# raider99k/UNINA-YOLO-DLA

Measured on AMD Instinct MI355X. Metric: frames/sec, 640x640 batch-1 (p99 latency alongside), higher is better.
Workload: dtype f16; 1 GPU; unina-yolo-dla-m graph A fp16, batch=1, 640x640, NMS on-GPU (BASELINE configs[1]); frames_in_flight_per_gpu=2, parallelism=1 GPU, distinct_frames=2048, detections_last_frame=446

## Files before the change

### include/unina_mi355.h

```cpp
#ifndef UNINA_MI355_H
#define UNINA_MI355_H

#include <stddef.h>
#include <stdint.h>

#ifdef UNINA_NO_HIP_HEADERS
typedef struct ihipStream_t *hipStream_t;
typedef int hipError_t;
#else
#include <hip/hip_runtime_api.h>
#endif

#ifdef __cplusplus
extern "C" {
#endif

#define MAX_DETECTIONS 1024

#if defined(__cplusplus)
struct alignas(32) GpuDetection {
#else
struct GpuDetection {
#endif
  float x1, y1, x2, y2;
// ... 275 lines not shown


typedef struct unina_op_info {
  char name[96];
  char kernel[64];
  int kind;
  int m, n, k;
  double flops;
  double bytes;
  int grid, block;
} unina_op_info;

int unina_op_count(const unina_engine_t *e);
int unina_get_op_info(const unina_engine_t *e, int index, unina_op_info *info);

int unina_profile_ops(unina_engine_t *e, int iters, float *ms_per_op, hipStream_t stream);

int unina_profile_post(unina_engine_t *e, int iters, float conf_threshold, float iou_threshold, float conformal_q, float *ms2,
                       hipStream_t stream);

int unina_conv_config_count(void);
const char *unina_conv_config_name(int cfg);
int unina_set_op_config(unina_engine_t *e, int op_index, int cfg);
int unina_autotune(unina_engine_t *e, int iters, hipStream_t stream);

int unina_set_fusion(unina_engine_t *e, int enable);
int unina_fusion_groups(const unina_engine_t *e);
int unina_debug_fusable_groups(const char *path);

int unina_debug_read_buffer(unina_engine_t *e, const char *name, float *host_out, size_t capacity_floats,
                            int *c, int *h, int *w);

int unina_debug_post_stamps(unina_engine_t *e, long long *out16);

int unina_debug_conv_stamps(unina_engine_t *e, int op_index, long long *out5, hipStream_t stream);

int unina_debug_dual_stamps(unina_engine_t *e, int op_index, long long *out16, hipStream_t stream);
int unina_debug_dual_timeline(unina_engine_t* e, int op_index, long long* out, int cap, hipStream_t stream);
int unina_debug_block_stamps(unina_engine_t *e, int op_index, long long *out16, hipStream_t stream);
int unina_debug_folded_heads(unina_engine_t *e);
int unina_debug_owned_streams(void);
int unina_debug_streams_overlap(int device, hipStream_t a, hipStream_t b, int reps, long long *stamps, int *overlapped);

const char *unina_version(void);

#define UNINA_COMM_ID_BYTES 128
typedef struct unina_comm unina_comm;
int unina_comm_unique_id(void *id128);
int unina_comm_init(unina_comm **out, const void *id128, int rank, int world, int device_id);
int unina_comm_all_gather(unina_comm *c, const void *d_send, void *d_recv, size_t bytes_per_rank, hipStream_t stream);
int unina_comm_rank(const unina_comm *c);
int unina_comm_world(const unina_comm *c);
void unina_comm_destroy(unina_comm *c);
const char *unina_comm_last_error(void);

hipError_t init_postprocess_resources(void);
hipError_t cleanup_postprocess_resources(void);
hipError_t reset_detection_counter(hipStream_t stream);
hipError_t get_detection_count(int *count, hipStream_t stream);
hipError_t decode_yolo_head(const float *d_cls, const float *d_reg, GpuDetection *d_detections, int grid_w,
                            int grid_h, int stride, int num_classes, float conf_threshold, float conformal_q,
                            hipStream_t stream);
hipError_t run_gpu_nms(GpuDetection *d_detections, int num_detections, float iou_threshold, hipStream_t stream);
hipError_t copy_valid_detections_to_host(const GpuDetection *d_detections, GpuDetection *h_detections,
                                         int num_detections, int *out_valid_count, hipStream_t stream);

// ... 33 lines not shown
```

### unina-yolo-dla_amd/csrc/engine.hip

```cpp
#include <cstdarg>
#include <cstdio>
#include <atomic>
#include <chrono>
#include <climits>
#include <cstdlib>
#include <cstring>
#include <string>
#include <vector>

#include "calib.h"
#include "engine_format.h"
#include "engine_validate.h"
#include "kernels.h"
#include "mining.h"

using namespace unina;

static_assert(kMaxClasses == (uint32_t)kMaxNumClasses, "the validator's class-count limit is the post-process's class field");

hipError_t unina::kernels_init() {
  for (hipError_t (*init)() : {conv_init, c3k2_init, head_init, pair_init, block_dual_init, stem_pool_init, post_init, calib_init}) {
    const hipError_t e = init();
    if (e != hipSuccess) return e;
  }
// ... 1993 lines not shown
                                 int y_pitch, int uv_pitch, const unina_tile* tiles, int n_tiles, const NormParams* norm,
                                 float conf, float iou, float q, float merge_iou, GpuDetection* d_out, int* d_out_count,
                                 hipStream_t stream) {
  const unina_frame f = nv12_frame(d_y, d_uv, src_width, src_height, y_pitch, uv_pitch);
  return infer_tiled(e, "unina_infer_tiled_nv12", &f, tiles, n_tiles, norm, conf, iou, q, merge_iou, true, d_out, d_out_count, stream);
}

int unina_infer_tiled_nv12(unina_engine_t* e, const uint8_t* d_y, const uint8_t* d_uv, int src_width, int src_height, int y_pitch,
                           int uv_pitch, const unina_tile* tiles, int n_tiles, const NormParams* norm, float conf, float iou,
                           float q, float merge_iou, GpuDetection* out, int* out_count, hipStream_t stream) {
  const unina_frame f = nv12_frame(d_y, d_uv, src_width, src_height, y_pitch, uv_pitch);
  return infer_tiled(e, "unina_infer_tiled_nv12", &f, tiles, n_tiles, norm, conf, iou, q, merge_iou, false, out, out_count, stream);
}

int unina_infer_tiled_frame_async(unina_engine_t* e, const unina_frame* frame, const unina_tile* tiles, int n_tiles, const NormParams* norm,
                                  float conf, float iou, float q, float merge_iou, GpuDetection* d_out, int* d_out_count,
                                  hipStream_t stream) {
  return infer_tiled(e, "unina_infer_tiled_frame_async", frame, tiles, n_tiles, norm, conf, iou, q, merge_iou, true, d_out, d_out_count, stream);
}

int unina_infer_tiled_frame(unina_engine_t* e, const unina_frame* frame, const unina_tile* tiles, int n_tiles, const NormParams* norm,
                            float conf, float iou, float q, float merge_iou, GpuDetection* out, int* out_count, hipStream_t stream) {
  return infer_tiled(e, "unina_infer_tiled_frame", frame, tiles, n_tiles, norm, conf, iou, q, merge_iou, false, out, out_count, stream);
}

int unina_debug_post_stamps(unina_engine_t* e, long long* out16) {
  if (!e || !out16) return UNINA_ERR_ARG;
  HIPCHK(e, hipSetDevice(e->device));
  HIPCHK(e, hipDeviceSynchronize());
  HIPCHK(e, hipMemcpy(out16, e->d_result->pad_stamps, sizeof(long long) * 16, hipMemcpyDeviceToHost));
  return UNINA_OK;
}

int unina_debug_conv_stamps(unina_engine_t* e, int op_index, long long* out5, hipStream_t stream) {
  if (!e || !out5 || op_index < 0 || op_index >= (int)e->ops.size()) return UNINA_ERR_ARG;
  HIPCHK(e, hipSetDevice(e->device));
  if (e->plan_dirty) {
    int rc = plan(e);
    if (rc != UNINA_OK) return rc;
  }
  if (e->ops[op_index].d.kind != kOpConv) return fail(e, UNINA_ERR_ARG, "op %d is not a convolution", op_index);
  long long* stamps = reinterpret_cast<long long*>(e->d_result->pad_stamps);
  HIPCHK(e, hipMemsetAsync(stamps, 0, sizeof(long long) * 8, stream));
  HIPCHK(e, launch_op_as(e, op_index, stream, kLaunchConv, [&](OpLaunch& l) { l.cp[0].stamps = stamps; }));
  HIPCHK(e, hipStreamSynchronize(stream));
  HIPCHK(e, hipMemcpy(out5, stamps, sizeof(long long) * 8, hipMemcpyDeviceToHost));
  return UNINA_OK;
}

int unina_debug_dual_stamps(unina_engine_t* e, int op_index, long long* out16, hipStream_t stream) {
  if (!e || !out16 || op_index < 0 || op_index >= (int)e->ops.size()) return UNINA_ERR_ARG;
  HIPCHK(e, hipSetDevice(e->device));
  if (e->plan_dirty) {
    int rc = plan(e);
    if (rc != UNINA_OK) return rc;
  }
  const PlannedOp& op = e->ops[op_index];
  if (op.d.kind != kOpConv || op.fuse_role || op.dual_with < 0 || op.dual_absorbed)
    return fail(e, UNINA_ERR_ARG, "op %d does not lead a dual conv launch", op_index);
  long long* stamps = reinterpret_cast<long long*>(e->d_result->pad_stamps);
  HIPCHK(e, hipMemsetAsync(stamps, 0, sizeof(long long) * 16, stream));
  HIPCHK(e, launch_op_as(e, op_index, stream, kLaunchConvDual, [&](OpLaunch& l) {
    l.cp[0].stamps = stamps;
    l.cp[1].stamps = stamps + 8;
  }));
  HIPCHK(e, hipStreamSynchronize(stream));
// ... 269 lines not shown
```

### unina-yolo-dla_amd/csrc/kernels.h

```cpp
#pragma once
#include <hip/hip_runtime.h>
#include <cstdint>
#include <vector>

#include "../../include/unina_mi355.h"
#include "camera_source.h"

namespace unina {

typedef _Float16 half_t;
enum DType : int { kF16 = 0, kF32 = 1, kI8 = 2, kS16 = 3 };
constexpr int kNumDTypes = 4;
struct s16_t { _Float16 v; };

struct LaunchDesc {
  const void* func;
  dim3 grid, block;
  unsigned shmem;
  const char* name;
};
inline hipError_t launch_desc(const LaunchDesc& d, void** args, hipStream_t stream) {
  return hipLaunchKernel(d.func, d.grid, d.block, args, d.shmem, stream);
}

// ... 195 lines not shown
  void* buf;
  long long lo;
  int H, W, C, ld, coff;
};
hipError_t sppf_pool_desc(const PoolParams& p, LaunchDesc* d);

struct QuantParams {
  const half_t* src;
  signed char* dst;
  size_t n;
  float inv_scale;
};
hipError_t quant_desc(const QuantParams& p, LaunchDesc* d);

struct CandList {
  GpuDetection* cand;
  uint2* ke;
  int* hist;
  int* total;
};
enum PostMode { kPostOneLaunch = 0, kPostSplit = 1 };
enum PostStamp {
  kStampDecoded = 0,
  kStampHandoff = 1, kStampListRead = 1,
  kStampGathered = 2,
  kStampSorted = 3, kStampNmsStart = 3,
  kStampMasks = 4, kStampTilesDone = 4,
  kStampScanned = 5,
  kStampOutput = 6,
  kStampDecodeStart = 7,
  kStampLoaded = 8,
  kStampLists = 9,
  kStampScanWave0 = 10,
  kPostStampCount = 14
};
struct PostParams {
  const float* cls[3];
  const float* reg[3];
  int gw[3], gh[3], stride[3];
  int num_classes;
  float conf_thr, iou_thr, conformal_q;
  GpuDetection* cand;
  int* block_count;
  unsigned int* ticket;
  GpuDetection* out;
  int* out_count;
  int* out_candidates;
  long long* stamps;
  unsigned int* done_flag;
  unsigned int done_value;
  PostMode mode;
  CandList list;
  float4* ws_box;
  float2* ws_cc;
  unsigned int* ticket2;
  int eoff[3];
  int* ws_rank;
  unsigned long long* ws_full;
  unsigned long long* ws_rownz;
  const void* h1[3];
  long long h1_lo[3];
  int h1_ld[3], h1_c[3];
  int h1_coff[3][2];
  const unsigned char* w2[3][2];
  const float* b2[3][2];
  int bstart[4];
  int cpb[3];
// ... 27 lines not shown
```

### unina-yolo-dla_amd/csrc/postprocess.hip

```cpp
#include "kernels.h"
#include "mfma_common.h"
#include "post_math.h"
#include "wave_block.h"

#pragma clang fp contract(off)

namespace unina {

namespace {

constexpr int kT = kPostBlock;
constexpr int kWaves = kT / 64;
constexpr int kMaxDet = MAX_DETECTIONS;
constexpr int kWords = kMaxDet / 64;
constexpr int kTriWords = 64 * (kWords * (kWords + 1) / 2);

struct Smem {
  int scan[kT + 8];
  unsigned long long keys[kMaxDet];
  float4 box[kMaxDet];
  float2 cc[kMaxDet];
  unsigned long long mask[kTriWords];
  unsigned long long rownz[kWords];
  unsigned long long removed[kWords];
// ... 438 lines not shown

namespace {

constexpr int kT2 = kPost2Block;
constexpr int kW2 = kT2 / 64;

struct SmemD {
  float stage[32][kT2];
  int wave_cnt[kW2];
  int run0;
};

constexpr int kTN = 512;
constexpr int kWN = kTN / 64;
constexpr int kColsPerWave = 64 / kWN;
constexpr int kMemCap = 1024;
struct SelectScratch {
  int hist[kBins];
  unsigned mkey[kMemCap];
  int meidx[kMemCap];
  int mpos[kMemCap];
  int part[kTN];
};
struct SmemN {
  float4 rbox[64], cbox[64];
  float2 rcc[64], ccc[64];
  unsigned char piece[64][kWN];
  unsigned char rcnt[64][kWN];
  union {
    unsigned long long mask[kMaxDet * kWords];
    SelectScratch sel;
  };
  unsigned short perm[kMaxDet];
  unsigned short list[4][kMaxDet];
  unsigned long long removed[4][kWords];
  unsigned long long rownz[kWords];
  int misc[4];
  int wave_cnt[kWN];
  int sel_cnt[kWN];
  int is_last;
};
static_assert(sizeof(SelectScratch) <= sizeof(unsigned long long) * kMaxDet * kWords, "select_top's scratch lives in the mask's LDS");
static_assert(kClassMask == kMaxNumClasses, "the all-ones class field is the dummy's -1");

__device__ __forceinline__ int list_reserve(const CandList& l, int count) {
  return count ? __hip_atomic_fetch_add(l.total, count, __ATOMIC_RELAXED, __HIP_MEMORY_SCOPE_AGENT) : 0;
}
__device__ __forceinline__ void list_put(const CandList& l, int at, uint4 box, uint4 rest, unsigned eidx) {
  uint4* dst = reinterpret_cast<uint4*>(l.cand + at);
  dst[0] = box;
  dst[1] = make_uint4(rest.x, rest.y, rest.z, eidx);
  l.ke[at] = make_uint2(rest.x, eidx);
  const int bin = conf_bin(__uint_as_float(rest.x));
  atomicAdd(&l.hist[bin < 0 ? 0 : bin], 1);
}

}

__global__ __launch_bounds__(kPost2Block) void post_decode_kernel(const PostParams p) {
  SmemD& s = *reinterpret_cast<SmemD*>(post_smem);
  const int tid = threadIdx.x, lane = tid & 63, wv = tid >> 6;
  const int b = blockIdx.x;
  const int h = b < p.bstart[1] ? 0 : (b < p.bstart[2] ? 1 : 2);
  const int cpb = p.cpb[h];
  const int cell0 = (b - p.bstart[h]) * cpb;
  const int gw = p.gw[h], ncell = gw * p.gh[h];
  const int idx = cell0 + tid;
  stamp(p.stamps, kStampDecodeStart, true);
  bool pass = false;
// ... 261 lines not shown
    st_sc1(p.ws_cc + c * 64 + tid, s.rcc[tid]);
  }
  const int gi = c * 64 + lane;
  const float4 a = s.rbox[lane];
  const float2 ac = s.rcc[lane];
  const float area_a = (a.z - a.x) * (a.w - a.y);
  unsigned int rowbits = 0u;
  int rowcnt = 0, colcnt = 0;
  unsigned long long colword = 0ull;
#pragma unroll
  for (int u = 0; u < kColsPerWave; ++u) {
    const int col = wv * kColsPerWave + u;
    const int gj = w * 64 + col;
    const float4 bb = s.cbox[col];
    const float2 bc = s.ccc[col];
    const bool j_first = bc.x > ac.x || (bc.x == ac.x && ce_eidx(bc.y) < ce_eidx(ac.y));
    const bool i_first = gi != gj && !j_first;
    const bool over = gi != gj && ce_same_class(bc.y, ac.y) && iou_exceeds(a, area_a, bb, p.iou_thr);
    if (over && ac.x > bc.x) rowbits |= 1u << u;
    rowcnt += j_first ? 1 : 0;
    const unsigned long long cw = __ballot(over && bc.x > ac.x);
    const int cc = __popcll(__ballot(i_first));
    if (lane == u) {
      colword = cw;
      colcnt = cc;
    }
  }
  s.piece[lane][wv] = (unsigned char)rowbits;
  s.rcnt[lane][wv] = (unsigned char)rowcnt;
  const unsigned long long colnz = __ballot(lane < kColsPerWave && colword != 0ull);
  if (w != c) {
    if (lane < kColsPerWave) {
      const int gj = w * 64 + wv * kColsPerWave + lane;
      st_sc1(p.ws_full + (size_t)gj * kWords + c, colword);
      atomicAdd(&p.ws_rank[gj], colcnt);
    }
    if (lane == 0 && colnz) atomicOr(&p.ws_rownz[w], colnz << (kColsPerWave * wv));
  }
  __syncthreads();
  if (tid < 64) {
    unsigned long long word = 0ull;
    int cnt = 0;
#pragma unroll
    for (int v = 0; v < kWN; ++v) {
      word |= (unsigned long long)s.piece[tid][v] << (kColsPerWave * v);
      cnt += s.rcnt[tid][v];
    }
    st_sc1(p.ws_full + (size_t)gi * kWords + w, word);
    atomicAdd(&p.ws_rank[gi], cnt);
    const unsigned long long nz = __ballot(word != 0ull);
    if (tid == 0 && nz) atomicOr(&p.ws_rownz[c], nz);
  }
}

struct OwnCands {
  int rk[2];
  float2 cc[2];
  float4 bx[2];
};

__device__ __forceinline__ OwnCands load_ranks_and_masks(SmemN& s, const PostParams& p, int n, int nw) {
  const int tid = threadIdx.x;
  constexpr int B = 8;
  const int words = n * nw;
  OwnCands o;
#pragma unroll
  for (int q = 0; q < 2; ++q) {
    const int e = tid + q * kTN;
    o.rk[q] = e < n ? __hip_atomic_load(p.ws_rank + e, __ATOMIC_RELAXED, __HIP_MEMORY_SCOPE_AGENT) : 0;
    o.cc[q] = e < n ? ld_sc1(p.ws_cc + e) : make_float2(0.f, 0.f);
    o.bx[q] = e < n ? ld_sc1(p.ws_box + e) : make_float4(0.f, 0.f, 0.f, 0.f);
  }
  unsigned long long rz = tid < kWords ? __hip_atomic_load(p.ws_rownz + tid, __ATOMIC_RELAXED, __HIP_MEMORY_SCOPE_AGENT) : 0ull;
  for (int k0 = tid; k0 < words; k0 += kTN * B) {
    unsigned long long v[B];
#pragma unroll
    for (int q = 0; q < B; ++q) {
      const int k = k0 + q * kTN;
      const int row = k / nw, wd = k - row * nw;
      v[q] = k < words ? ld_sc1(p.ws_full + (size_t)row * kWords + wd) : 0ull;
    }
#pragma unroll
    for (int q = 0; q < B; ++q) {
      const int k = k0 + q * kTN;
      if (k < words) s.mask[k] = v[q];
    }
  }
  if (tid < kWords) s.rownz[tid] = rz;
  __syncthreads();
#pragma unroll
  for (int q = 0; q < 2; ++q) {
    const int e = tid + q * kTN;
    if (e < n && (unsigned)o.rk[q] < (unsigned)n) {
      const unsigned nz = (unsigned)((s.rownz[e >> 6] >> (e & 63)) & 1ull);
      s.perm[o.rk[q]] = (unsigned short)(e | ((__float_as_int(o.cc[q].y) & 3) << 10) | (nz << 12));
    }
  }
  __syncthreads();
  return o;
}

__device__ __forceinline__ void class_split_scan(SmemN& s, long long* stamps, int n, int nw) {
  const int tid = threadIdx.x, lane = tid & 63, wv = tid >> 6;
  if (wv < 4) {
    unsigned long long removed_reg = 0ull;
    int m = 0;
    for (int r0 = 0; r0 < n; r0 += 64) {
      const int r = r0 + lane;
      const int ent = r < n ? (int)s.perm[r] : 0;
      const bool take = r < n && (ent >> 12) && ((ent >> 10) & 3) == wv;
      const unsigned long long bal = __ballot(take);
      if (take) s.list[wv][m + __popcll(bal & ((1ull << lane) - 1ull))] = (unsigned short)(ent & 1023);
      m += __popcll(bal);
    }
    asm volatile("s_waitcnt lgkmcnt(0)" ::: "memory");
    stamp(stamps, kStampLists);
    if (stamps && lane == 0) stamps[kStampScanWave0 + wv] = m;
    for (int k0 = 0; k0 < m; k0 += 64) {
      const int cnt = m - k0 < 64 ? m - k0 : 64;
      const int mine = k0 + lane < m ? (int)s.list[wv][k0 + lane] : 0;
      for (int kb = 0; kb < cnt; kb += 16) {
        unsigned long long pre[16];
#pragma unroll
        for (int q = 0; q < 16; ++q) {
          const int iq = __builtin_amdgcn_readlane(mine, (kb + q) & 63);
          pre[q] = lane < nw ? s.mask[iq * nw + lane] : 0ull;
        }
#pragma unroll
        for (int q = 0; q < 16; ++q) {
          const int i = __builtin_amdgcn_readlane(mine, (kb + q) & 63);
          const unsigned long long cur = lane_word(removed_reg, i >> 6);
          const bool act = kb + q < cnt && !((cur >> (i & 63)) & 1ull);
          removed_reg |= act ? pre[q] : 0ull;
        }
      }
    }
    if (lane < kWords) s.removed[wv][lane] = removed_reg;
    if (stamps && lane == 0) stamps[kStampScanWave0 + wv] |= (long long)(wall_clock64() & 0xFFFFFFFFll) << 20;
  }
  __syncthreads();
  if (tid < kWords) s.removed[0][tid] |= s.removed[1][tid] | s.removed[2][tid] | s.removed[3][tid];
  __syncthreads();
}

__device__ __forceinline__ void emit_and_reset(SmemN& s, const PostParams& p, int n, int nw, int total, const OwnCands& o) {
  const int tid = threadIdx.x;
  int base = 0;
#pragma unroll
  for (int q = 0; q < 2; ++q) {
    const int r = tid + q * kTN;
    if (q * kTN >= n) break;
    bool kept = false;
    if (r < n) {
      const int i = s.perm[r] & 1023;
      kept = !((s.removed[0][i >> 6] >> (i & 63)) & 1ull);
    }
    int tot;
    const int at = base + block_rank<kWN>(kept, s.wave_cnt, &tot);
    if (r < n) s.list[0][r] = (unsigned short)at;
    base += tot;
  }
  __syncthreads();
#pragma unroll
  for (int q = 0; q < 2; ++q) {
    const int e = tid + q * kTN;
    if (e < n && (unsigned)o.rk[q] < (unsigned)n && !((s.removed[0][e >> 6] >> (e & 63)) & 1ull)) {
      GpuDetection d = make_det(o.bx[q], o.cc[q].x, ce_class(o.cc[q].y), 1);
      map_box(p, d);
      p.out[s.list[0][o.rk[q]]] = d;
    }
  }
  for (int e = tid; e < nw * 64; e += kTN) p.ws_rank[e] = 0;
  if (tid < kWords) p.ws_rownz[tid] = 0ull;
  for (int i = tid; i < kBins; i += kTN) p.list.hist[i] = 0;
  if (tid == 0) {
    *p.out_count = base;
    if (p.out_candidates) *p.out_candidates = total;
    __hip_atomic_store(p.list.total, 0, __ATOMIC_RELAXED, __HIP_MEMORY_SCOPE_AGENT);
    __hip_atomic_store(p.ticket2, 0u, __ATOMIC_RELAXED, __HIP_MEMORY_SCOPE_AGENT);
  }
}

}

__global__ __launch_bounds__(kTN) void post_nms_kernel(const PostParams p) {
  SmemN& s = *reinterpret_cast<SmemN*>(post_smem);
  stamp(p.stamps, kStampNmsStart, true);
  const int total = __hip_atomic_load(p.list.total, __ATOMIC_RELAXED, __HIP_MEMORY_SCOPE_AGENT);
  stamp(p.stamps, kStampListRead, true);
  const int n = total < kMaxDet ? total : kMaxDet;
  const int nw = (n + 63) >> 6;
  const int ntiles = nw * (nw + 1) / 2;
  const int t = blockIdx.x;
  if (t >= (ntiles > 0 ? ntiles : 1)) return;
  if (ntiles > 0) {
    const TileCW tile = tile_of(t, nw);
    fetch_tile(s, p, total, n, tile);
    stamp(p.stamps, kStampGathered, true);
    pair_tile(s, p, tile);
    if (!arrive_and_check_last_sc1(p.ticket2, &s.is_last, ntiles)) return;
  }
  stamp(p.stamps, kStampTilesDone);
  const OwnCands own = load_ranks_and_masks(s, p, n, nw);
  stamp(p.stamps, kStampLoaded);
  class_split_scan(s, p.stamps, n, nw);
  stamp(p.stamps, kStampScanned);
  emit_and_reset(s, p, n, nw, total, own);
  stamp(p.stamps, kStampOutput);
  signal_done(p, threadIdx.x);
}

__global__ __launch_bounds__(kPost2Block) void tile_gather_kernel(const TileGatherParams g) {
  int& s_base = *reinterpret_cast<int*>(post_smem);
  const int t = blockIdx.x, tid = threadIdx.x;
  int cnt = g.counts[t];
  cnt = cnt < 0 ? 0 : (cnt > kMaxDet ? kMaxDet : cnt);
  if (tid == 0) s_base = list_reserve(g.list, cnt);
  __syncthreads();
  const int base = s_base;
  const TileMap m = g.map[t];
  const uint4* src = reinterpret_cast<const uint4*>(g.slots + (size_t)t * kMaxDet);
  for (int i = tid; i < cnt; i += kPost2Block) {
    const uint4 bx = src[2 * i], rest = src[2 * i + 1];
    const float x1 = __uint_as_float(bx.x) * m.sx + m.ox, y1 = __uint_as_float(bx.y) * m.sy + m.oy;
    const float x2 = __uint_as_float(bx.z) * m.sx + m.ox, y2 = __uint_as_float(bx.w) * m.sy + m.oy;
    list_put(g.list, base + i, make_uint4(__float_as_uint(x1), __float_as_uint(y1), __float_as_uint(x2), __float_as_uint(y2)), rest,
             (unsigned)(t * kMaxDet + i));
  }
}

int post_num_blocks(const int gw[3], const int gh[3]) {
  const int cells = gw[0] * gh[0] + gw[1] * gh[1] + gw[2] * gh[2];
  return (cells + kPostBlock - 1) / kPostBlock;
}

constexpr size_t kListCap = 256 * 1024;
static_assert(kListCap == (size_t)1 << (32 - kClassBits), "an enumeration index must fit the bits above the class in pack_ce");
size_t post_workspace_bytes() {
  return sizeof(float4) * kMaxDet + sizeof(float2) * kMaxDet + 256 + sizeof(int) * kBins + sizeof(uint2) * kListCap +
         sizeof(int) * kMaxDet + sizeof(unsigned long long) * ((size_t)kMaxDet * kWords + kWords);
// ... 237 lines not shown
```

### unina-yolo-dla_amd/engine.py

```python
from __future__ import annotations

import ctypes as C
import os
import tempfile
from typing import Dict, List, Optional

import numpy as np

from . import export as _export
from .graph import Graph, OUTPUT_NAMES

_PKG = os.path.dirname(os.path.abspath(__file__))
LIB_PATH = os.environ.get("UNINA_LIB") or os.path.join(_PKG, "libunina_mi355.so")
MAX_DETECTIONS = 1024

DET_DTYPE = np.dtype([("x1", "<f4"), ("y1", "<f4"), ("x2", "<f4"), ("y2", "<f4"), ("confidence", "<f4"),
                      ("class_id", "<i4"), ("valid", "<i4"), ("_pad", "<i4")])
assert DET_DTYPE.itemsize == 32

ERRORS = {1: "IO", 2: "FORMAT", 3: "HIP", 4: "ARG", 5: "STATE", 6: "UNSUPPORTED"}


class OpInfo(C.Structure):
    _fields_ = [("name", C.c_char * 96), ("kernel", C.c_char * 64), ("kind", C.c_int), ("m", C.c_int), ("n", C.c_int),
# ... 120 lines not shown

CLUSTER_DTYPE = np.dtype([(n, "<f4") for n in ("x", "y", "z_lo", "z_hi", "x_lo", "x_hi", "y_lo", "y_hi")] +
                         [(n, "<i4") for n in ("n_points", "n_cells", "root", "cone")])
CLUSTER_HEADER_DTYPE = np.dtype([(n, "<i4") for n in ("n_points", "n_in_grid", "n_cells", "n_components", "n_cones", "n_written", "n_dropped",
                                                      "reserved")])
assert CLUSTER_DTYPE.itemsize == 48 and CLUSTER_HEADER_DTYPE.itemsize == 32


class ClusterParams(C.Structure):
    _fields_ = [("x_min", C.c_float), ("y_min", C.c_float), ("cell", C.c_float), ("nx", C.c_int), ("ny", C.c_int), ("min_points", C.c_int),
                ("max_points", C.c_int), ("min_height", C.c_float), ("max_height", C.c_float), ("max_width", C.c_float),
                ("confidence", C.c_float), ("class_id", C.c_int)]


class TrackParams(C.Structure):
    _fields_ = [("pose", C.c_float * 12), ("gate", C.c_float), ("alpha", C.c_float), ("birth_confidence", C.c_float),
                ("class_aware", C.c_int), ("confirm_hits", C.c_int), ("max_missed", C.c_int)]


def _tile_array(tiles):
    return (Tile * len(tiles))(*[Tile(*map(int, t)) for t in tiles])


class EngineError(RuntimeError):
    pass


_lib: Optional[C.CDLL] = None

ABI_SYMBOLS = [
    "unina_load_engine", "unina_unload_engine", "unina_engine_input_dims", "unina_set_tensor_address",
    "unina_tensor_address", "unina_enqueue", "unina_infer", "unina_infer_bgra", "unina_infer_nv12", "unina_infer_async", "unina_postprocess_async",
    "unina_last_error", "unina_op_count", "unina_get_op_info", "unina_profile_ops", "unina_profile_post", "unina_debug_read_buffer",
    "unina_version", "unina_conv_config_count", "unina_conv_config_name", "unina_set_op_config", "unina_autotune", "unina_debug_post_stamps", "unina_debug_conv_stamps", "unina_debug_dual_stamps", "unina_debug_dual_timeline", "unina_debug_block_stamps", "unina_debug_folded_heads", "unina_serial_latency",
    "unina_debug_owned_streams", "unina_debug_streams_overlap",
    "unina_set_fusion", "unina_fusion_groups", "unina_debug_fusable_groups",
    "unina_slice_tiles", "unina_infer_tiled_bgra", "unina_infer_tiled_bgra_async", "unina_merge_tiles_async",
    "unina_infer_tiled_nv12", "unina_infer_tiled_nv12_async", "unina_preprocess_nv12_resize",
    "unina_letterbox_geometry", "unina_infer_letterbox_bgra", "unina_infer_letterbox_nv12", "unina_infer_letterbox_bgra_async",
    "unina_infer_letterbox_nv12_async", "unina_preprocess_letterbox_bgra", "unina_preprocess_letterbox_nv12",
    "unina_infer_frame", "unina_infer_frame_async", "unina_infer_letterbox_frame", "unina_infer_letterbox_frame_async",
    "unina_infer_tiled_frame", "unina_infer_tiled_frame_async", "unina_preprocess_frame", "unina_preprocess_letterbox_frame",
    "unina_embedding_dim", "unina_mine_async", "unina_mine", "unina_mine_heads_async", "unina_kcenter",
    "unina_kmeans_workspace_bytes", "unina_kmeans", "unina_nearest_rows",
    "unina_abs_histogram_f16", "unina_calib_buffer_count", "unina_calib_buffer_name", "unina_calib_buffers_async", "unina_calib_async",
    "unina_eval_create", "unina_eval_destroy", "unina_eval_reset_async", "unina_eval_update_async", "unina_eval_read",
    "unina_locate_async", "unina_locate_stereo_async", "unina_rectify_async",
    "unina_lidar_create", "unina_lidar_destroy", "unina_locate_lidar_async", "unina_lidar_buffers",
    "unina_ground_create", "unina_ground_destroy", "unina_ground_filter_async", "unina_ground_buffers",
    "unina_cluster_create", "unina_cluster_destroy", "unina_cluster_async", "unina_cluster_buffers",
    "unina_track_create", "unina_track_destroy", "unina_track_reset_async", "unina_track_update_async", "unina_track_buffers",
    "unina_track_read",
    "unina_comm_unique_id", "unina_comm_init", "unina_comm_all_gather", "unina_comm_rank", "unina_comm_world", "unina_comm_destroy",
    "unina_comm_last_error",
    "create_norm_params_imagenet", "create_norm_params", "preprocess_bgra_resize", "preprocess_bgra", "preprocess_nv12",
    "allocate_preprocess_buffer", "free_preprocess_buffer", "create_preprocess_stream", "destroy_preprocess_stream",
    "init_postprocess_resources", "cleanup_postprocess_resources", "reset_detection_counter", "get_detection_count",
    "decode_yolo_head", "run_gpu_nms", "copy_valid_detections_to_host",
]


def load_library() -> C.CDLL:
    global _lib
    if _lib is not None:
        return _lib
    if not os.path.exists(LIB_PATH):
        raise EngineError(f"{LIB_PATH} is missing: build it with __graft_entry__.build() "
                          f"(hipcc --offload-arch=gfx950). There is no CPU fallback.")
    L = C.CDLL(LIB_PATH)
    vp, ci, cf = C.c_void_p, C.c_int, C.c_float
    L.unina_load_engine.argtypes = [C.c_char_p, ci, C.POINTER(vp)]
    L.unina_unload_engine.argtypes = [vp]
    L.unina_unload_engine.restype = None
    L.unina_engine_input_dims.argtypes = [vp, C.POINTER(ci), C.POINTER(ci), C.POINTER(ci)]
    L.unina_set_tensor_address.argtypes = [vp, C.c_char_p, vp]
    L.unina_tensor_address.argtypes = [vp, C.c_char_p, C.POINTER(vp), C.POINTER(C.c_size_t)]
    L.unina_enqueue.argtypes = [vp, vp]
    L.unina_infer.argtypes = [vp, vp, cf, cf, cf, vp, C.POINTER(ci), vp]
    L.unina_infer_async.argtypes = [vp, vp, cf, cf, cf, vp, vp, vp]
    L.unina_infer_bgra.argtypes = [vp, vp, ci, ci, ci, C.POINTER(NormParams), cf, cf, cf, vp, C.POINTER(ci), vp]
    L.unina_infer_nv12.argtypes = [vp, vp, vp, ci, ci, ci, ci, C.POINTER(NormParams), cf, cf, cf, vp, C.POINTER(ci), vp]
    L.unina_postprocess_async.argtypes = [vp, cf, cf, cf, vp, vp, vp]
    L.unina_last_error.argtypes = [vp]
    L.unina_last_error.restype = C.c_char_p
    L.unina_op_count.argtypes = [vp]
    L.unina_get_op_info.argtypes = [vp, ci, C.POINTER(OpInfo)]
    L.unina_profile_ops.argtypes = [vp, ci, C.POINTER(cf), vp]
    L.unina_profile_post.argtypes = [vp, ci, cf, cf, cf, C.POINTER(cf), vp]
    L.unina_debug_read_buffer.argtypes = [vp, C.c_char_p, vp, C.c_size_t, C.POINTER(ci), C.POINTER(ci), C.POINTER(ci)]
    L.unina_version.restype = C.c_char_p
    L.unina_conv_config_name.restype = C.c_char_p
    L.unina_conv_config_name.argtypes = [ci]
    L.unina_set_op_config.argtypes = [vp, ci, ci]
    L.unina_autotune.argtypes = [vp, ci, vp]
    L.unina_set_fusion.argtypes = [vp, ci]
    L.unina_fusion_groups.argtypes = [vp]
    L.unina_debug_fusable_groups.argtypes = [C.c_char_p]
    L.unina_debug_post_stamps.argtypes = [vp, C.POINTER(C.c_longlong)]
    L.unina_debug_conv_stamps.argtypes = [vp, ci, C.POINTER(C.c_longlong), vp]
    L.unina_debug_dual_stamps.argtypes = [vp, ci, C.POINTER(C.c_longlong), vp]
    L.unina_debug_dual_timeline.argtypes = [vp, ci, C.POINTER(C.c_longlong), ci, vp]
    L.unina_debug_block_stamps.argtypes = [vp, ci, C.POINTER(C.c_longlong), vp]
    L.unina_debug_folded_heads.argtypes = [vp]
    L.unina_debug_owned_streams.argtypes = []
    L.unina_debug_streams_overlap.argtypes = [ci, vp, vp, ci, C.POINTER(C.c_longlong), C.POINTER(ci)]
    L.unina_serial_latency.argtypes = [vp, C.POINTER(vp), ci, ci, cf, cf, cf, C.POINTER(C.c_double), vp]
    L.unina_slice_tiles.argtypes = [ci, ci, ci, ci, cf, cf, C.POINTER(Tile), ci]
    L.unina_infer_tiled_bgra.argtypes = [vp, vp, ci, ci, ci, C.POINTER(Tile), ci, C.POINTER(NormParams), cf, cf, cf, cf, vp,
                                         C.POINTER(ci), vp]
    L.unina_infer_tiled_bgra_async.argtypes = [vp, vp, ci, ci, ci, C.POINTER(Tile), ci, C.POINTER(NormParams), cf, cf, cf, cf, vp,
                                               vp, vp]
    L.unina_infer_tiled_nv12.argtypes = [vp, vp, vp, ci, ci, ci, ci, C.POINTER(Tile), ci, C.POINTER(NormParams), cf, cf, cf, cf, vp,
                                         C.POINTER(ci), vp]
    L.unina_infer_tiled_nv12_async.argtypes = [vp, vp, vp, ci, ci, ci, ci, C.POINTER(Tile), ci, C.POINTER(NormParams), cf, cf, cf, cf,
                                               vp, vp, vp]
    L.unina_merge_tiles_async.argtypes = [vp, vp, vp, C.POINTER(Tile), ci, cf, vp, vp, vp]
    L.unina_letterbox_geometry.argtypes = [ci, ci, ci, ci, C.POINTER(Letterbox)]
    L.unina_infer_letterbox_bgra.argtypes = [vp, vp, ci, ci, ci, C.POINTER(NormParams), cf, cf, cf, cf, ci, vp, C.POINTER(ci), vp]
    L.unina_infer_letterbox_bgra_async.argtypes = [vp, vp, ci, ci, ci, C.POINTER(NormParams), cf, cf, cf, cf, ci, vp, vp, vp]
    L.unina_infer_letterbox_nv12.argtypes = [vp, vp, vp, ci, ci, ci, ci, C.POINTER(NormParams), cf, cf, cf, cf, ci, vp,
                                             C.POINTER(ci), vp]
    L.unina_infer_letterbox_nv12_async.argtypes = [vp, vp, vp, ci, ci, ci, ci, C.POINTER(NormParams), cf, cf, cf, cf, ci, vp, vp, vp]
    L.unina_preprocess_letterbox_bgra.argtypes = [vp, vp, ci, ci, ci, ci, ci, cf, NormParams, vp]
    L.unina_preprocess_letterbox_nv12.argtypes = [vp, vp, vp, ci, ci, ci, ci, ci, ci, cf, NormParams, vp]
    fp, npp = C.POINTER(Frame), C.POINTER(NormParams)
    L.unina_infer_frame.argtypes = [vp, fp, npp, cf, cf, cf, vp, C.POINTER(ci), vp]
    L.unina_infer_frame_async.argtypes = [vp, fp, npp, cf, cf, cf, vp, vp, vp]
    L.unina_infer_letterbox_frame.argtypes = [vp, fp, npp, cf, cf, cf, cf, ci, vp, C.POINTER(ci), vp]
    L.unina_infer_letterbox_frame_async.argtypes = [vp, fp, npp, cf, cf, cf, cf, ci, vp, vp, vp]
    L.unina_infer_tiled_frame.argtypes = [vp, fp, C.POINTER(Tile), ci, npp, cf, cf, cf, cf, vp, C.POINTER(ci), vp]
    L.unina_infer_tiled_frame_async.argtypes = [vp, fp, C.POINTER(Tile), ci, npp, cf, cf, cf, cf, vp, vp, vp]
# ... 430 lines not shown
    def autotune(self, images=None, iters: int = 10, stream=None, cache: Optional[str] = None) -> None:
        import json
        names = self.conv_configs()
        key = f"{self.width}x{self.height}:{self.op_infos()[1]['kernel'][:13]}:" + "|".join(f"{o['m']},{o['n']},{o['k']}" for o in self.op_infos())
        if cache and os.path.exists(cache):
            try:
                with open(cache) as f:
                    blob = json.load(f)
                if blob.get("key") == key and blob.get("configs") == names:
                    for i, c in enumerate(blob["choice"]):
                        if c >= 0:
                            self.set_op_config(i, c)
                    return
            except (ValueError, KeyError):
                pass
        if images is None and self._images is None:
            images = _torch().zeros((1, 3, self.height, self.width), dtype=_torch().float32,
                                    device=_torch().device("cuda", self.device))
        if images is not None:
            self.bind_images(images)
        self._check(self.L.unina_autotune(self.h, iters, _stream_ptr(stream)))
        _torch().cuda.synchronize(self.device)
        if cache:
            norm = [o["kernel"].replace("<f32,", "<f16,") for o in self.op_infos()]
            choice = [names.index(k) if k in names else -1 for k in norm]
            with open(cache, "w") as f:
                json.dump({"key": key, "configs": names, "choice": choice}, f)

    def debug_stamps(self):
        buf = (C.c_longlong * 16)()
        self._check(self.L.unina_debug_post_stamps(self.h, buf))
        return [int(v) for v in buf]

    def conv_stamps(self, op_index: int, stream=None) -> List[int]:
        buf = (C.c_longlong * 8)()
        self._check(self.L.unina_debug_conv_stamps(self.h, op_index, buf, _stream_ptr(stream)))
        return [int(v) for v in buf]

    def dual_stamps(self, op_index: int, stream=None) -> List[int]:
        buf = (C.c_longlong * 16)()
        self._check(self.L.unina_debug_dual_stamps(self.h, op_index, buf, _stream_ptr(stream)))
        return [int(v) for v in buf]

    def block_stamps(self, op_index: int, stream=None) -> List[int]:
        buf = (C.c_longlong * 16)()
        self._check(self.L.unina_debug_block_stamps(self.h, op_index, buf, _stream_ptr(stream)))
        return [int(v) for v in buf]

    def dual_timeline(self, op_index: int, stream=None):
        cap = 2 * 4096 + 2
        buf = (C.c_longlong * cap)()
        n = self.L.unina_debug_dual_timeline(self.h, op_index, buf, cap, _stream_ptr(stream))
        if n <= 0:
            raise RuntimeError(f"unina_debug_dual_timeline: error {-n}")
        return np.array(buf[:2 * n + 2], dtype=np.int64).reshape(n + 1, 2)

    def folded_heads(self) -> List[bool]:
        m = self.L.unina_debug_folded_heads(self.h)
        if m < 0:
            raise EngineError(f"[{ERRORS.get(-m, -m)}] unina_debug_folded_heads")
        return [bool(m >> h & 1) for h in range(3)]

    def conv_configs(self) -> List[str]:
        return [self.L.unina_conv_config_name(i).decode() for i in range(self.L.unina_conv_config_count())]

    def set_op_config(self, op_index: int, cfg: int) -> bool:
# ... 265 lines not shown
```

Before: 10100 frames/s.

## Replace class-split NMS scan with single-wave bitset scan over marking rows

The on-GPU NMS now gathers only the candidates whose suppression rows are nonzero (marking rows) in rank order, and loads just those rows of the IoU bitmask. The old four-wave per-class list scan is replaced by one wave that resolves suppression with ballots over 16-row batches. The suppression workspace is written only where a word is nonzero and cleared only at the nonzero entries, cutting global stores and the reset cost. The single-wave scan gives up the 4-way class parallelism and adds extra syncs, and correctness depends on the sparse writes always being matched by the sparse reset. A debug entry point that counts nonzero workspace words is added to check this.

```diff
diff --git a/include/unina_mi355.h b/include/unina_mi355.h
--- a/include/unina_mi355.h
+++ b/include/unina_mi355.h
@@ -331,6 +331,8 @@
                             int *c, int *h, int *w);
 
 int unina_debug_post_stamps(unina_engine_t *e, long long *out16);
+
+int unina_debug_post_workspace_nonzero(unina_engine_t *e, int *out3);
 
 int unina_debug_conv_stamps(unina_engine_t *e, int op_index, long long *out5, hipStream_t stream);
 
diff --git a/unina-yolo-dla_amd/csrc/engine.hip b/unina-yolo-dla_amd/csrc/engine.hip
--- a/unina-yolo-dla_amd/csrc/engine.hip
+++ b/unina-yolo-dla_amd/csrc/engine.hip
@@ -2049,6 +2049,25 @@
   return UNINA_OK;
 }
 
+int unina_debug_post_workspace_nonzero(unina_engine_t* e, int* out3) {
+  if (!e || !out3 || !e->d_post_ws) return UNINA_ERR_ARG;
+  HIPCHK(e, hipSetDevice(e->device));
+  HIPCHK(e, hipDeviceSynchronize());
+  PostParams pp;
+  memset(&pp, 0, sizeof pp);
+  post_bind_workspace(&pp, e->d_post_ws, e->d_cand);
+  const size_t nfull = (size_t)MAX_DETECTIONS * (MAX_DETECTIONS / 64), nnz = MAX_DETECTIONS / 64;
+  std::vector<unsigned long long> words(nfull + nnz);
+  std::vector<int> rank(MAX_DETECTIONS);
+  HIPCHK(e, hipMemcpy(words.data(), pp.ws_full, sizeof(unsigned long long) * nfull, hipMemcpyDeviceToHost));
+  HIPCHK(e, hipMemcpy(words.data() + nfull, pp.ws_rownz, sizeof(unsigned long long) * nnz, hipMemcpyDeviceToHost));
+  HIPCHK(e, hipMemcpy(rank.data(), pp.ws_rank, sizeof(int) * MAX_DETECTIONS, hipMemcpyDeviceToHost));
+  out3[0] = out3[1] = out3[2] = 0;
+  for (size_t i = 0; i < nfull + nnz; ++i) out3[i < nfull ? 0 : 1] += words[i] != 0ull;
+  for (int v : rank) out3[2] += v != 0;
+  return UNINA_OK;
+}
+
 int unina_debug_conv_stamps(unina_engine_t* e, int op_index, long long* out5, hipStream_t stream) {
   if (!e || !out5 || op_index < 0 || op_index >= (int)e->ops.size()) return UNINA_ERR_ARG;
   HIPCHK(e, hipSetDevice(e->device));
diff --git a/unina-yolo-dla_amd/csrc/kernels.h b/unina-yolo-dla_amd/csrc/kernels.h
--- a/unina-yolo-dla_amd/csrc/kernels.h
+++ b/unina-yolo-dla_amd/csrc/kernels.h
@@ -251,7 +251,8 @@
   kStampLoaded = 8,
   kStampLists = 9,
   kStampScanWave0 = 10,
-  kPostStampCount = 14
+  kStampMarking = 14,
+  kPostStampCount = 15
 };
 struct PostParams {
   const float* cls[3];
diff --git a/unina-yolo-dla_amd/csrc/postprocess.hip b/unina-yolo-dla_amd/csrc/postprocess.hip
--- a/unina-yolo-dla_amd/csrc/postprocess.hip
+++ b/unina-yolo-dla_amd/csrc/postprocess.hip
@@ -494,9 +494,9 @@
     SelectScratch sel;
   };
   unsigned short perm[kMaxDet];
-  unsigned short list[4][kMaxDet];
-  unsigned long long removed[4][kWords];
-  unsigned long long rownz[kWords];
+  unsigned short mrow[kMaxDet];
+  unsigned short opos[kMaxDet];
+  unsigned long long removed[kWords];
   int misc[4];
   int wave_cnt[kWN];
   int sel_cnt[kWN];
@@ -824,7 +824,7 @@
   if (w != c) {
     if (lane < kColsPerWave) {
       const int gj = w * 64 + wv * kColsPerWave + lane;
-      st_sc1(p.ws_full + (size_t)gj * kWords + c, colword);
+      if (colword != 0ull) st_sc1(p.ws_full + (size_t)gj * kWords + c, colword);
       atomicAdd(&p.ws_rank[gj], colcnt);
     }
     if (lane == 0 && colnz) atomicOr(&p.ws_rownz[w], colnz << (kColsPerWave * wv));
@@ -838,7 +838,7 @@
       word |= (unsigned long long)s.piece[tid][v] << (kColsPerWave * v);
       cnt += s.rcnt[tid][v];
     }
-    st_sc1(p.ws_full + (size_t)gi * kWords + w, word);
+    if (word != 0ull) st_sc1(p.ws_full + (size_t)gi * kWords + w, word);
     atomicAdd(&p.ws_rank[gi], cnt);
     const unsigned long long nz = __ballot(word != 0ull);
     if (tid == 0 && nz) atomicOr(&p.ws_rownz[c], nz);
@@ -851,10 +851,9 @@
   float4 bx[2];
 };
 
-__device__ __forceinline__ OwnCands load_ranks_and_masks(SmemN& s, const PostParams& p, int n, int nw) {
-  const int tid = threadIdx.x;
+__device__ __forceinline__ OwnCands load_ranks_and_marking_rows(SmemN& s, const PostParams& p, int n, int nw, int* nmark) {
+  const int tid = threadIdx.x, lane = tid & 63, wv = tid >> 6;
   constexpr int B = 8;
-  const int words = n * nw;
   OwnCands o;
 #pragma unroll
   for (int q = 0; q < 2; ++q) {
@@ -863,14 +862,36 @@
     o.cc[q] = e < n ? ld_sc1(p.ws_cc + e) : make_float2(0.f, 0.f);
     o.bx[q] = e < n ? ld_sc1(p.ws_box + e) : make_float4(0.f, 0.f, 0.f, 0.f);
   }
-  unsigned long long rz = tid < kWords ? __hip_atomic_load(p.ws_rownz + tid, __ATOMIC_RELAXED, __HIP_MEMORY_SCOPE_AGENT) : 0ull;
+  const unsigned long long rz = lane < kWords ? __hip_atomic_load(p.ws_rownz + lane, __ATOMIC_RELAXED, __HIP_MEMORY_SCOPE_AGENT) : 0ull;
+#pragma unroll
+  for (int q = 0; q < 2; ++q) {
+    const int e = tid + q * kTN;
+    const unsigned nz = (unsigned)((lane_word(rz, wv + q * kWN) >> lane) & 1ull);
+    if (e < n && (unsigned)o.rk[q] < (unsigned)n)
+      s.perm[o.rk[q]] = (unsigned short)(e | (nz << 12));
+  }
+  __syncthreads();
+  int R = 0;
+#pragma unroll
+  for (int q = 0; q < 2; ++q) {
+    const int r = tid + q * kTN;
+    if (q * kTN >= n) break;
+    const int ent = r < n ? (int)s.perm[r] : 0;
+    int tot;
+    const int at = R + block_rank<kWN>((ent >> 12) != 0, s.wave_cnt, &tot);
+    if (ent >> 12) s.mrow[at] = (unsigned short)(ent & 1023);
+    R += tot;
+  }
+  __syncthreads();
+  stamp(p.stamps, kStampMarking);
+  const int words = R * nw;
   for (int k0 = tid; k0 < words; k0 += kTN * B) {
     unsigned long long v[B];
 #pragma unroll
     for (int q = 0; q < B; ++q) {
       const int k = k0 + q * kTN;
       const int row = k / nw, wd = k - row * nw;
-      v[q] = k < words ? ld_sc1(p.ws_full + (size_t)row * kWords + wd) : 0ull;
+      v[q] = k < words ? ld_sc1(p.ws_full + (size_t)s.mrow[k < words ? row : 0] * kWords + wd) : 0ull;
     }
 #pragma unroll
     for (int q = 0; q < B; ++q) {
@@ -878,64 +899,68 @@
       if (k < words) s.mask[k] = v[q];
     }
   }
-  if (tid < kWords) s.rownz[tid] = rz;
-  __syncthreads();
-#pragma unroll
-  for (int q = 0; q < 2; ++q) {
-    const int e = tid + q * kTN;
-    if (e < n && (unsigned)o.rk[q] < (unsigned)n) {
-      const unsigned nz = (unsigned)((s.rownz[e >> 6] >> (e & 63)) & 1ull);
-      s.perm[o.rk[q]] = (unsigned short)(e | ((__float_as_int(o.cc[q].y) & 3) << 10) | (nz << 12));
-    }
-  }
-  __syncthreads();
+  __syncthreads();
+  *nmark = R;
   return o;
 }
 
-__device__ __forceinline__ void class_split_scan(SmemN& s, long long* stamps, int n, int nw) {
+__device__ __forceinline__ void bitset_scan(SmemN& s, long long* stamps, int R, int nw) {
   const int tid = threadIdx.x, lane = tid & 63, wv = tid >> 6;
-  if (wv < 4) {
-    unsigned long long removed_reg = 0ull;
-    int m = 0;
-    for (int r0 = 0; r0 < n; r0 += 64) {
-      const int r = r0 + lane;
-      const int ent = r < n ? (int)s.perm[r] : 0;
-      const bool take = r < n && (ent >> 12) && ((ent >> 10) & 3) == wv;
-      const unsigned long long bal = __ballot(take);
-      if (take) s.list[wv][m + __popcll(bal & ((1ull << lane) - 1ull))] = (unsigned short)(ent & 1023);
-      m += __popcll(bal);
-    }
-    asm volatile("s_waitcnt lgkmcnt(0)" ::: "memory");
+  R = __builtin_amdgcn_readfirstlane(R);
+  nw = __builtin_amdgcn_readfirstlane(nw);
+  if (wv == 0) {
     stamp(stamps, kStampLists);
-    if (stamps && lane == 0) stamps[kStampScanWave0 + wv] = m;
-    for (int k0 = 0; k0 < m; k0 += 64) {
-      const int cnt = m - k0 < 64 ? m - k0 : 64;
-      const int mine = k0 + lane < m ? (int)s.list[wv][k0 + lane] : 0;
-      for (int kb = 0; kb < cnt; kb += 16) {
-        unsigned long long pre[16];
+    const int sub = lane >> 4, w = lane & 15;
+    const unsigned* half = reinterpret_cast<const unsigned*>(s.mask);
+    unsigned long long acc = 0ull;
+    for (int k0 = 0; k0 < R; k0 += 64) {
+      const int cnt = R - k0 < 64 ? R - k0 : 64;
+      const bool in = lane < cnt;
+      const int pos = in ? (int)s.mrow[k0 + lane] : 0;
+      const int pw = pos >> 6, pb = pos & 63;
+      const int ph = pos >> 5;
+      const unsigned bit = in ? 1u << (pos & 31) : 0u;
+      const unsigned long long seen = ((unsigned long long)(unsigned)__shfl((int)(unsigned)(acc >> 32), pw) << 32) |
+                                      (unsigned)__shfl((int)(unsigned)acc, pw);
+      unsigned long long dead = __ballot(in && ((seen >> pb) & 1ull));
+#pragma unroll
+      for (int kb = 0; kb < 64; kb += 16) {
+        if (kb >= cnt) break;
+        unsigned pre[16];
 #pragma unroll
         for (int q = 0; q < 16; ++q) {
-          const int iq = __builtin_amdgcn_readlane(mine, (kb + q) & 63);
-          pre[q] = lane < nw ? s.mask[iq * nw + lane] : 0ull;
+          const int k = kb + q < cnt ? kb + q : cnt - 1;
+          pre[q] = half[2 * (k0 + k) * nw + ph];
         }
 #pragma unroll
         for (int q = 0; q < 16; ++q) {
-          const int i = __builtin_amdgcn_readlane(mine, (kb + q) & 63);
-          const unsigned long long cur = lane_word(removed_reg, i >> 6);
-          const bool act = kb + q < cnt && !((cur >> (i & 63)) & 1ull);
-          removed_reg |= act ? pre[q] : 0ull;
+          const unsigned long long dep = __ballot((pre[q] & bit) != 0u);
+          dead |= ((dead >> (kb + q)) & 1ull) ? 0ull : dep;
         }
       }
-    }
-    if (lane < kWords) s.removed[wv][lane] = removed_reg;
-    if (stamps && lane == 0) stamps[kStampScanWave0 + wv] |= (long long)(wall_clock64() & 0xFFFFFFFFll) << 20;
-  }
-  __syncthreads();
-  if (tid < kWords) s.removed[0][tid] |= s.removed[1][tid] | s.removed[2][tid] | s.removed[3][tid];
-  __syncthreads();
-}
-
-__device__ __forceinline__ void emit_and_reset(SmemN& s, const PostParams& p, int n, int nw, int total, const OwnCands& o) {
+      for (int k4 = 0; k4 < cnt; k4 += 16) {
+        unsigned long long m[4];
+#pragma unroll
+        for (int q = 0; q < 4; ++q) {
+          const int k = k4 + 4 * q + sub;
+          const bool take = k < cnt && w < nw && !((dead >> k) & 1ull);
+          m[q] = take ? s.mask[(k0 + k) * nw + w] : 0ull;
+        }
+        acc |= (m[0] | m[1]) | (m[2] | m[3]);
+      }
+#pragma unroll
+      for (int j = 16; j <= 32; j <<= 1)
+        acc |= ((unsigned long long)(unsigned)__shfl_xor((int)(unsigned)(acc >> 32), j) << 32) | (unsigned)__shfl_xor((int)(unsigned)acc, j);
+    }
+    if (lane < kWords) s.removed[lane] = acc;
+    if (stamps && lane == 0) {
+      for (int v = 0; v < 4; ++v) stamps[kStampScanWave0 + v] = (v == 0 ? R : 0) | ((long long)(wall_clock64() & 0xFFFFFFFFll) << 20);
+    }
+  }
+  __syncthreads();
+}
+
+__device__ __forceinline__ void emit_and_reset(SmemN& s, const PostParams& p, int n, int nw, int total, int R, const OwnCands& o) {
   const int tid = threadIdx.x;
   int base = 0;
 #pragma unroll
@@ -945,22 +970,26 @@
     bool kept = false;
     if (r < n) {
       const int i = s.perm[r] & 1023;
-      kept = !((s.removed[0][i >> 6] >> (i & 63)) & 1ull);
+      kept = !((s.removed[i >> 6] >> (i & 63)) & 1ull);
     }
     int tot;
     const int at = base + block_rank<kWN>(kept, s.wave_cnt, &tot);
-    if (r < n) s.list[0][r] = (unsigned short)at;
+    if (r < n) s.opos[r] = (unsigned short)at;
     base += tot;
   }
   __syncthreads();
 #pragma unroll
   for (int q = 0; q < 2; ++q) {
     const int e = tid + q * kTN;
-    if (e < n && (unsigned)o.rk[q] < (unsigned)n && !((s.removed[0][e >> 6] >> (e & 63)) & 1ull)) {
+    if (e < n && (unsigned)o.rk[q] < (unsigned)n && !((s.removed[e >> 6] >> (e & 63)) & 1ull)) {
       GpuDetection d = make_det(o.bx[q], o.cc[q].x, ce_class(o.cc[q].y), 1);
       map_box(p, d);
-      p.out[s.list[0][o.rk[q]]] = d;
-    }
+      p.out[s.opos[o.rk[q]]] = d;
+    }
+  }
+  for (int k = tid; k < R * kWords; k += kTN) {
+    const int row = k / kWords, wd = k % kWords;
+    if (wd < nw && s.mask[row * nw + wd] != 0ull) p.ws_full[(size_t)s.mrow[row] * kWords + wd] = 0ull;
   }
   for (int e = tid; e < nw * 64; e += kTN) p.ws_rank[e] = 0;
   if (tid < kWords) p.ws_rownz[tid] = 0ull;
@@ -993,11 +1022,12 @@
     if (!arrive_and_check_last_sc1(p.ticket2, &s.is_last, ntiles)) return;
   }
   stamp(p.stamps, kStampTilesDone);
-  const OwnCands own = load_ranks_and_masks(s, p, n, nw);
+  int R;
+  const OwnCands own = load_ranks_and_marking_rows(s, p, n, nw, &R);
   stamp(p.stamps, kStampLoaded);
-  class_split_scan(s, p.stamps, n, nw);
+  bitset_scan(s, p.stamps, R, nw);
   stamp(p.stamps, kStampScanned);
-  emit_and_reset(s, p, n, nw, total, own);
+  emit_and_reset(s, p, n, nw, total, R, own);
   stamp(p.stamps, kStampOutput);
   signal_done(p, threadIdx.x);
 }
diff --git a/unina-yolo-dla_amd/engine.py b/unina-yolo-dla_amd/engine.py
--- a/unina-yolo-dla_amd/engine.py
+++ b/unina-yolo-dla_amd/engine.py
@@ -176,7 +176,7 @@
     "unina_load_engine", "unina_unload_engine", "unina_engine_input_dims", "unina_set_tensor_address",
     "unina_tensor_address", "unina_enqueue", "unina_infer", "unina_infer_bgra", "unina_infer_nv12", "unina_infer_async", "unina_postprocess_async",
     "unina_last_error", "unina_op_count", "unina_get_op_info", "unina_profile_ops", "unina_profile_post", "unina_debug_read_buffer",
-    "unina_version", "unina_conv_config_count", "unina_conv_config_name", "unina_set_op_config", "unina_autotune", "unina_debug_post_stamps", "unina_debug_conv_stamps", "unina_debug_dual_stamps", "unina_debug_dual_timeline", "unina_debug_block_stamps", "unina_debug_folded_heads", "unina_serial_latency",
+    "unina_version", "unina_conv_config_count", "unina_conv_config_name", "unina_set_op_config", "unina_autotune", "unina_debug_post_stamps", "unina_debug_post_workspace_nonzero", "unina_debug_conv_stamps", "unina_debug_dual_stamps", "unina_debug_dual_timeline", "unina_debug_block_stamps", "unina_debug_folded_heads", "unina_serial_latency",
     "unina_debug_owned_streams", "unina_debug_streams_overlap",
     "unina_set_fusion", "unina_fusion_groups", "unina_debug_fusable_groups",
     "unina_slice_tiles", "unina_infer_tiled_bgra", "unina_infer_tiled_bgra_async", "unina_merge_tiles_async",
@@ -241,6 +241,7 @@
     L.unina_fusion_groups.argtypes = [vp]
     L.unina_debug_fusable_groups.argtypes = [C.c_char_p]
     L.unina_debug_post_stamps.argtypes = [vp, C.POINTER(C.c_longlong)]
+    L.unina_debug_post_workspace_nonzero.argtypes = [vp, C.POINTER(ci)]
     L.unina_debug_conv_stamps.argtypes = [vp, ci, C.POINTER(C.c_longlong), vp]
     L.unina_debug_dual_stamps.argtypes = [vp, ci, C.POINTER(C.c_longlong), vp]
     L.unina_debug_dual_timeline.argtypes = [vp, ci, C.POINTER(C.c_longlong), ci, vp]
@@ -737,6 +738,11 @@
         self._check(self.L.unina_debug_post_stamps(self.h, buf))
         return [int(v) for v in buf]
 
+    def post_workspace_nonzero(self) -> List[int]:
+        buf = (C.c_int * 3)()
+        self._check(self.L.unina_debug_post_workspace_nonzero(self.h, buf))
+        return [int(v) for v in buf]
+
     def conv_stamps(self, op_index: int, stream=None) -> List[int]:
         buf = (C.c_longlong * 8)()
         self._check(self.L.unina_debug_conv_stamps(self.h, op_index, buf, _stream_ptr(stream)))
```

Measured after the change: 10100 frames/s (median of 3 runs). About the same (-0.0%).
